# Photoroom/datago

Hardware: AMD Instinct MI355X
Metric: Mpixel/s device-resident JPEG decode+bucket-resize at 1/2/4/8 MI355X (higher is better)
Workload: dtype u8

## Files before the change

datago_amd/csrc/dg_entropy.h:

```cpp
#pragma once
#include "dg_pixel.h"
#include "dg_plane.h"
#include "dg_types.h"

namespace dg {

DG_HD int32_t huff_extend(int32_t v, int32_t s) { return v < (1 << (s - 1)) ? v - (1 << s) + 1 : v; }

DG_HD uint32_t bswap32(uint32_t x) {
  return (x >> 24) | ((x >> 8) & 0xFF00u) | ((x << 8) & 0xFF0000u) | (x << 24);
}

DG_HD uint32_t ds_word_index(uint32_t w, uint32_t lsw) {
  const uint32_t s = w >> lsw, j = w & ((1u << lsw) - 1u);
  return ((((s >> 6) << lsw) + j) << 6) + (s & 63u);
}
DG_HD uint64_t ds_words_alloc(uint32_t nsub, uint32_t lsw) {
  const uint32_t margin = ((1024u >> 5) >> lsw) + 2u;
  return ((uint64_t)((nsub + margin + 63u) / 64u) << lsw) * 64;
}

constexpr uint32_t kBwBuf = 6;

struct BitWin {
// ... 98 lines not shown
      eob = 1;
      break;
    }
    const uint32_t nadv = adv + (size == 0u ? 16u : run + 1u);
    if (nadv > 64u) break;
    adv = nadv;
    o += len + size;
    if (adv == 64u) break;
  }
  return o | (adv << 4) | (eob << 11);
}

DG_HD uint32_t multi_next_z(uint32_t m, uint32_t z) {
  const uint32_t c = m & 15u, adv = (m >> 4) & 127u, eob = (m >> 11) & 1u;
  const bool ok = c != 0u && z != 0u && (eob ? z + adv < 64u : z + adv <= 64u);
  return ok ? (eob ? 64u : z + adv) : 0xFFFFFFFFu;
}

struct RangeAcc {
  uint32_t out;
  uint32_t m, n;
  int32_t dc[3];
};

struct WriteCtx {
  int16_t *blk;
  uint32_t sw = 0;
  DG_GLOBAL int16_t *coef;
  uint32_t seg, nin;
  int32_t pred[3];
  uint32_t blocks_per_seg, total_blocks;
  int32_t cur;
  uint32_t zs;
#if defined(DG_DEVICE)
  DG_GLOBAL uint8_t *cnt = nullptr;
  int16_t *wave_blk;
  uint32_t stride;
  uint32_t *tab;
  const ImageDesc *im;
  const int32_t *qt;
  const uint8_t *n2z;
  BatchFlags *flags;
  uint32_t img;
#endif
};

DG_HD int32_t wc_index(const WriteCtx &w, uint32_t in_seg) {
  if (w.blocks_per_seg && in_seg >= w.blocks_per_seg) return -1;
  uint64_t g = (uint64_t)(w.blocks_per_seg ? w.seg : 0) * w.blocks_per_seg + in_seg;
  return g < w.total_blocks ? (int32_t)g : -1;
}

DG_HD void wc_begin(WriteCtx &w, int32_t idx, uint32_t zs) {
  w.cur = idx;
  w.zs = zs;
#if defined(DG_DEVICE)
  u32x4 *p = (u32x4 *)w.blk;
  const u32x4 zero = {0u, 0u, 0u, 0u};
#pragma unroll
  for (int i = 0; i < 8; i++) p[i] = zero;
#else
  for (int i = 0; i < 64; i++) w.blk[i] = 0;
#endif
}

DG_HD void wc_flush(WriteCtx &w, uint32_t ze) {
  if (w.cur < 0) return;
  DG_GLOBAL int16_t *dst = w.coef + (size_t)w.cur * 64;
  if (w.zs == 0 && ze == 64) {
#if defined(DG_DEVICE)
    const u32x4 *s4 = (const u32x4 *)w.blk;
    DG_GLOBAL u32x4 *d4 = (DG_GLOBAL u32x4 *)dst;
#pragma unroll
    for (int i = 0; i < 8; i++) d4[i] = s4[i ^ (w.sw >> 3)];
#else
    for (int i = 0; i < 64; i++) dst[i] = w.blk[i ^ w.sw];
#endif
  } else {
    for (uint32_t i = w.zs; i < ze; i++) dst[i] = w.blk[i ^ w.sw];
  }
#if defined(DG_DEVICE)
  if (w.cnt) w.cnt[w.cur] = 0xFFu;
#endif
  w.cur = -1;
}

#if defined(DG_DEVICE)
__device__ __forceinline__ void wc_list_late(WriteCtx &w, int32_t idx) {
  if (!w.im || idx < 0) return;
  const uint32_t e = atomicAdd(&w.flags->idct_late, 1u);
  if (e < w.flags->idct_cap) {
    uint32_t *l = (uint32_t *)(uintptr_t)w.flags->idct_list;
    l[2 * e] = w.img;
    l[2 * e + 1] = (uint32_t)idx;
  }
}

__device__ __forceinline__ void wc_coop_flush(WriteCtx &w, bool pending) {
  const uint64_t pm = __ballot(pending);
  if (!pm) return;
  const uint64_t am = __ballot(1);
  if (pending) {
    const uint32_t rank = __builtin_amdgcn_mbcnt_hi((uint32_t)(pm >> 32), __builtin_amdgcn_mbcnt_lo((uint32_t)pm, 0u));
    w.tab[rank] = __lane_id();
    w.tab[64 + rank] = (uint32_t)w.cur;
  }
  __builtin_amdgcn_wave_barrier();
  const uint32_t wr = __builtin_amdgcn_mbcnt_hi((uint32_t)(am >> 32), __builtin_amdgcn_mbcnt_lo((uint32_t)am, 0u));
  const uint32_t na = (uint32_t)__popcll(am), nb = (uint32_t)__popcll(pm), nc = 8u * nb;
  const u32x4 zero = {0u, 0u, 0u, 0u};
  if (w.im && na >= 8) {
    const ImageDesc &im = *w.im;
    const bool zune = im.sem != 0;
    const uint32_t groups = na >> 3, g = wr >> 3, part = wr & 7u;
    for (uint32_t k0 = 0; k0 < nb; k0 += groups) {
      const uint32_t k = k0 + g;
      const bool act = g < groups && k < nb;
      const int32_t idx = act ? (int32_t)w.tab[64 + k] : -1;
      const uint32_t own = act ? w.tab[k] & 255u : 0u;
      int16_t *b = w.wave_blk + own * w.stride;
      const uint32_t osw = w.stride == 64u ? ((own >> 1) & 7u) << 3 : 0u;
      const bool live = act && idx >= 0;
      uint32_t c = 0, by = 0, bx = 0;
      if (live) block_pos(im, (uint32_t)idx, c, by, bx);
      int32_t ws[8];
      if (live) {
        int32_t v[8];
#pragma unroll
        for (int r = 0; r < 8; r++) v[r] = (int32_t)b[w.n2z[r * 8 + part] ^ osw] * w.qt[c * 64 + r * 8 + part];
        idct_col(zune, v, ws);
      }
      __builtin_amdgcn_wave_barrier();
      if (live) {
#pragma unroll
        for (int r = 0; r < 8; r++) b[r * 8 + part] = (int16_t)ws[r];
      }
      __builtin_amdgcn_wave_barrier();
      if (act) {
        u32x4 *row4 = (u32x4 *)b + part;
        if (live) {
          const u32x4 rv = *row4;
          int16_t h[8];
          __builtin_memcpy(h, &rv, 16);
          int32_t row[8];
          uint32_t px[8];
#pragma unroll
          for (int i = 0; i < 8; i++) row[i] = h[i];
          idct_row(zune, row, px);
          store_plane_row8(im, c, by * 8 + part, bx, px);
        }
        *row4 = zero;
      }
      __builtin_amdgcn_wave_barrier();
    }
    return;
  }
  for (uint32_t c = wr; c < nc; c += na) {
    const uint32_t k = c >> 3, part = c & 7u;
    const int32_t idx = (int32_t)w.tab[64 + k];
    const uint32_t own = w.tab[k] & 255u;
    u32x4 *src = (u32x4 *)(w.wave_blk + own * w.stride) + (w.stride == 64u ? part ^ ((own >> 1) & 7u) : part);
    const u32x4 v = *src;
    const bool nz = (v.x | v.y | v.z | v.w) != 0u;
    if (idx >= 0 && (nz || !w.cnt)) *(DG_GLOBAL u32x4 *)(w.coef + (size_t)idx * 64 + part * 8) = v;
    if (w.cnt && nz) atomicOr(&w.tab[k], 256u << part);
    *src = zero;
    if (part == 0) wc_list_late(w, idx);
  }
  __builtin_amdgcn_wave_barrier();
  if (w.cnt && wr < nb) {
    const int32_t idx = (int32_t)w.tab[64 + wr];
    if (idx >= 0) w.cnt[idx] = (uint8_t)(w.tab[wr] >> 8);
  }
  __builtin_amdgcn_wave_barrier();
}

__device__ __forceinline__ void wc_flush_zero(WriteCtx &w, uint32_t ze) {
  wc_flush(w, ze);
  u32x4 *p = (u32x4 *)w.blk;
  const u32x4 zero = {0u, 0u, 0u, 0u};
#pragma unroll
  for (int i = 0; i < 8; i++) p[i] = zero;
}
#endif

template <bool COOP>
DG_HD void wc_end_block(WriteCtx &w, bool &pending) {
// ... 282 lines not shown
    const int32_t v = huff_value(bits, len, size);
    uint32_t zm = 0xFFFFFFFFu, mc = 0;
    if (!WRITE) {
      const uint32_t m = (mi != 3u && !isdc) ? (uint32_t)mt[(mi << kMultiBits) | (bits >> (32u - kMultiBits))] : 0u;
      mc = m & 15u;
      zm = pos + mc <= ev ? multi_next_z(m, z) : 0xFFFFFFFFu;
    }
    const bool take_m = zm != 0xFFFFFFFFu;
    pos += take_m ? mc : len + size;
    const int32_t vdc = isdc ? v : 0;
    acc.n += isdc ? 1u : 0u;
    add3(acc.dc, comp, vdc);
    if (stage) {
      if (isdc) {
        stg->started++;
        if (v) stage_push(*stg, stage_coef(0, stg->started, v));
      } else if (size && z + run < 64) {
        stage_push(*stg, stage_coef(z + run, stg->started, v));
      }
    }
    if (WRITE) {
      add3(w->pred, comp, vdc);
      if (isdc) {
        if (COOP) {
          w->cur = wc_index(*w, w->nin);
          w->zs = 0;
        } else {
          wc_begin(*w, wc_index(*w, w->nin), 0);
        }
        w->nin++;
      }
      const uint32_t zz = z + run;
      if (isdc || (size && zz < 64u)) w->blk[zz ^ w->sw] = (int16_t)(isdc ? sel3(w->pred, comp) : v);
    }
    uint32_t zn = take_m ? zm : huff_next_z(z, sym);
    if (pair && !stage && (WRITE || !take_m)) {
      uint32_t used = len + size;
      bool open = isdc || !(size == 0u && run != 15u);
#pragma unroll
      for (uint32_t x = 0; x < 3u; x++) {
        if (x >= pair) break;
        const uint32_t bx = used < 32u ? bits << used : 0u;
        const uint32_t ex = huff_decode(*tac, bx);
        const uint32_t lx = ex >> 8, sx = ex & 0xFFu, zx = sx & 15u;
        const bool tk = open && zn < 64u && pos < ev && used + lx + zx <= 32u;
        if (tk) {
          if (WRITE) {
            const uint32_t zz2 = zn + (sx >> 4);
            if (zx && zz2 < 64u) w->blk[zz2 ^ w->sw] = (int16_t)huff_value(bx, lx, zx);
          }
          pos += lx + zx;
          used += lx + zx;
          zn = huff_next_z(zn, sx);
        }
        open = tk && !(zx == 0u && (sx >> 4) != 15u);
      }
    }
    bw_shift(b, pos);
    const bool bend = zn >= 64u;
    if (WRITE && bend) wc_end_block<COOP>(*w, pending);
    z = bend ? 0u : zn;
    r = bend ? (r + 1u == bpm ? 0u : r + 1u) : r;
    comp = (cbits >> (2u * r)) & 3u;
    block_tables(tdc, tac);
  }
  if (WRITE && z > 0) wc_partial<COOP>(*w, z);
  if (stage) stage_finish(*stg);
  if (!merged) {
    uint32_t rel = pos - a1;
    acc.out = pack_state(rel > 255 ? 255 : rel, r, z);
  }
  for (uint32_t j = 0; j < k; j++) {
    DG_GLOBAL Ckpt &c = ck[j];
    if (acc.m > c.m) {
      c.m = acc.m - c.m;
      c.n = acc.n;
      c.dc[0] = acc.dc[0];
      c.dc[1] = acc.dc[1];
      c.dc[2] = acc.dc[2];
    } else {
      c.m = 0;
      c.n = acc.n - c.n;
// ... 242 lines not shown
```

datago_amd/csrc/dg_types.h:

```cpp
#pragma once
#include <stdint.h>

#if defined(__HIP__)
#define DG_HD __host__ __device__ __forceinline__
#define DG_DEVICE 1
#define DG_GLOBAL __attribute__((address_space(1)))
typedef unsigned int u32x4 __attribute__((ext_vector_type(4)));
typedef unsigned int u32x2 __attribute__((ext_vector_type(2)));
#else
#define DG_HD static inline
#define DG_GLOBAL
#endif

namespace dg {

template <class T>
DG_HD DG_GLOBAL T *gp(uint64_t a) {
  return (DG_GLOBAL T *)(uintptr_t)a;
}

DG_HD int32_t sel3(const int32_t v[3], uint32_t c) { return c == 0 ? v[0] : (c == 1 ? v[1] : v[2]); }
DG_HD void add3(int32_t v[3], uint32_t c, int32_t d) {
  v[0] += c == 0 ? d : 0;
  v[1] += c == 1 ? d : 0;
// ... 10 lines not shown
constexpr int kSubBits = 16 - kLutBits;
constexpr int kMaxSubTables = 8;
struct HuffTable {
  uint16_t lut[1 << kLutBits];
  uint16_t sub[kMaxSubTables][1 << kSubBits];
  uint32_t lim[17];
  int32_t valoff[17];
  uint8_t vals[256];
};

struct QuantTable {
  uint16_t q[64];
};

DG_HD uint32_t pack_state(uint32_t rel, uint32_t r, uint32_t z) {
  return 0x80000000u | (rel << 16) | (r << 8) | z;
}
DG_HD uint32_t st_rel(uint32_t s) { return (s >> 16) & 0xFFu; }
DG_HD uint32_t st_r(uint32_t s) { return (s >> 8) & 0xFFu; }
DG_HD uint32_t st_z(uint32_t s) { return s & 0xFFu; }

struct SubState {
  uint32_t in;
  uint32_t out;
  uint32_t m;
  uint32_t n;
  int32_t dc[3];
  uint32_t seg;
  uint32_t nin;
  int32_t dcin[3];
  uint32_t nstart;
  uint32_t nent;
};

enum Colorspace : uint32_t { CS_YCC = 0, CS_RGB = 1, CS_GRAY = 2 };

struct ResizePass {
  uint64_t src, dst;
  uint64_t coef;
  uint64_t bounds;
  double in0, in1;
  uint32_t in_size, out_size;
  uint32_t ksize;
  int32_t precision;
  uint32_t src_stride, dst_stride;
  uint32_t width, rows;
  uint32_t out0;
  uint32_t bands;
  uint32_t row0;
  uint32_t C;
  uint32_t kind;
  uint32_t mode;
};
constexpr uint32_t kHFused = 1, kHDirect = 2;
constexpr uint32_t kHVFused = 4;
constexpr uint32_t kHDecode = 8, kHDecWide = 16;
constexpr uint32_t kDecCols = 128;
constexpr uint32_t kDecSeg0 = 320, kDecSeg1 = 640;
constexpr uint32_t kDecStripsDefault = 8;
constexpr uint32_t kHVSegPx = 320;
constexpr uint32_t kHVTapsMax = 24;
constexpr uint32_t kHVRows = 64;
constexpr uint32_t kHBandRows = 8;
constexpr uint32_t kHBandCols = 128;
constexpr uint32_t kIdctItemStride = 4;

// ... 109 lines not shown
  uint64_t scan;
  uint32_t scan_len;
  uint32_t nsub;
  uint32_t sub_base;
  uint32_t sub_bits;
  uint32_t ckpt_base;
  uint64_t ds;
  uint64_t mk;
  uint64_t chunk;
  uint32_t nchunk;
  uint32_t ds_state0;
  uint32_t ds_bits;
  uint32_t nmk;
  uint32_t slotmap;
  uint32_t mk_cap;
  uint32_t lead_bits;
  uint32_t ds_lsw;
  uint32_t ckpt;
  uint32_t idct_fused;
  uint32_t stage_cap;
  uint32_t restart;
  uint32_t blocks_per_seg;
  uint32_t total_blocks;
  uint32_t bpm;
  uint32_t comp_bits;
  uint8_t blk_comp[12];
  uint16_t hslot[kMaxSlots];
  uint8_t ncomp, colorspace, dec_c, nslots;
  uint16_t qpool[3];
  uint16_t sem;
  uint64_t coef;
  uint64_t stage;
  uint64_t ccnt;
  uint32_t width, height;
  uint32_t mcux, mcuy;
  uint32_t hmax, vmax;
  uint32_t ch[3], cv[3];
  uint32_t cfirst[3];
  uint32_t cbw[3], cbh[3];
  uint32_t cdsw[3], cdsh[3];
  uint64_t plane[3];
  uint64_t pix;
  uint32_t pix_stride;
  int32_t status;
  ResizePass pass[kStages];
  uint64_t out;
  uint32_t out_w, out_h, out_c, out_stride;
  uint64_t final_src;
  uint32_t final_src_stride, copy_needed;
  uint32_t final_src_c;
  uint32_t color_fused;
  uint32_t fmt;
  uint32_t prog;
  uint32_t crec;
  uint32_t copy_mode;
  PngDesc png;
  AlphaOp aop[kAlphaPoints];
  EncDesc enc;
};

struct ProgScan {
  uint64_t data;
  uint32_t len;
  uint32_t image;
  uint32_t ns;
  uint32_t comp[4];
// ... 42 lines not shown
```

datago_amd/csrc/host/pipeline.cpp:

```cpp
#include "pipeline.h"

#include <string.h>

#include <algorithm>
#include <time.h>
#include <atomic>
#include <chrono>
#include <cmath>
#include <thread>

#include "../dg_entropy.h"
#include "../dg_pixel.h"
#include "../kernels.h"

namespace dg {

thread_local std::string g_last_error;
void set_error(const std::string &s) { g_last_error = s; }

#define HIPCHK(x)                                                                          \
  do {                                                                                     \
    hipError_t e_ = (x);                                                                   \
    if (e_ != hipSuccess) {                                                                \
      set_error(std::string("HIP error: ") + hipGetErrorString(e_) + " at " #x);          \
// ... 492 lines not shown
    return DG_OK;
  }
  if (k == "prog_pipe") {
    prog_pipe_ = v != 0;
    return DG_OK;
  }
  if (k == "prog_serial") {
    prog_serial_ = v != 0;
    return DG_OK;
  }
  if (k == "entropy_once") {
    entropy_once_ = v != 0;
    return DG_OK;
  }
  if (k == "entropy_lpt") {
    entropy_lpt_ = v != 0;
    return DG_OK;
  }
  if (k == "hb_bands") {
    if (v < 1 || v > 64) return opt_error(k, v, "valid unless v < 1 || v > 64");
    hb_bands_ = (uint32_t)v;
    return DG_OK;
  }
  if (k == "idct_fused") {
    idct_fused_ = v != 0;
    return DG_OK;
  }
  if (k == "idct_thread") {
    idct_thread_ = v != 0;
    return DG_OK;
  }
  if (k == "sparse_coef") {
    sparse_coef_ = v != 0;
    return DG_OK;
  }
  if (k == "h_prefetch") {
    h_prefetch_ = v != 0;
    return DG_OK;
  }
  if (k == "h_planar") {
    h_planar_ = v != 0;
    return DG_OK;
  }
  if (k == "destuff_one") {
    destuff_one_ = v != 0;
    return DG_OK;
  }
  if (k == "chroma_rec") {
    chroma_rec_ = v != 0;
    return DG_OK;
  }
  if (k == "reset_host_us") {
    for (double &x : host_us_) x = 0;
    for (double &x : host_cpu_us_) x = 0;
    return DG_OK;
  }
  if (k == "hv_fused") {
    hv_fused_ = v != 0;
    return DG_OK;
  }
  if (k == "copy_threads") {
    if (v < 1 || v > 64) return opt_error(k, v, "valid unless v < 1 || v > 64");
    copy_threads_ = (int)v;
    return DG_OK;
  }
  if (k == "ckpt") {
// ... 870 lines not shown
  ccache_maybe_reset(sl);
  struct CacheRoll {
    Context *c;
    size_t n0, off0;
    bool armed = true;
    ~CacheRoll() {
      if (armed) c->ccache_rollback(n0, off0);
    }
  } croll{this, ccache_.size(), ccache_off_};
  uint32_t sub_bits = sub_bits_;
  bool small = false;
  if (!sub_bits) {
    uint64_t coded = 0;
    for (int i = 0; i < n; i++)
      if (!b.plans[i].status && b.plans[i].fmt == kFmtJpeg && !b.plans[i].hdr.progressive)
        coded += b.plans[i].hdr.scan_end - b.plans[i].hdr.scan_off;
    small = coded < small_coded_;
    sub_bits = coded >= (64ull << 20) ? sub_auto_ : small ? sub_small_ : 2048u;
  }
  last_sub_bits_ = sub_bits;
  Layout L;
  Layout CO;
  Layout IN;
  Layout LT, CH;
  const bool alias = png_alias_;
  std::vector<size_t> in_off(n, 0);
  size_t out_total = 0;
  uint64_t ckpt_total = 0;
  b.out_dev_off.assign(n, 0);
  b.out_direct.assign(n, 0);
  uint32_t sub_base = 0;
  b.descs.reserve(n);
  struct Offs {
    size_t coef, ccnt, plane[3], pix, pass_dst[kStages], pass_coef[kStages], pass_bounds[kStages], pass_srcoff[kStages];
    int pass_cache[kStages];
    bool pass_hit[kStages];
    size_t final_off, tmp, out, ds, mk, chunk, stage;
    size_t zs, raw, unf, pal;
    size_t tout, ecoef, ebits, ewords, hdr, eaux;
    int aop_stage[kAlphaPoints];
    size_t aop_off[kAlphaPoints];
    uint32_t late = 0;
    int img = -1;
  };
  std::vector<Offs> offs;
  for (int i = 0; i < n; i++) {
    ImagePlan &p = b.plans[i];
    if (p.status) continue;
    ImageDesc d;
    memset(&d, 0, sizeof(d));
    Offs o;
    memset(&o, 0, sizeof(o));
    o.late = 0;
    o.img = i;
    for (int s_ = 0; s_ < kStages; s_++) o.pass_cache[s_] = -1;
    uint32_t W, H, C;
    size_t cur_stride;
    bool colour = false;
    if (p.fmt == kFmtPng) {
      const PngHeader &g = p.png;
      W = g.width;
      H = g.height;
      C = (uint32_t)g.out_c;
      d.fmt = kFmtPng;
      d.width = W;
      d.height = H;
      d.dec_c = (uint8_t)C;
// ... 126 lines not shown
        d.sub_bits = sub_bits / 4;
      else if (bpb < sub_density_ && sub_bits >= 1024)
        d.sub_bits = sub_bits / 2;
    }
    d.idct_fused = (idct_fused_ && !entropy_once_) ? 1u : 0u;
    if (write_split_ && d.ckpt && !d.idct_fused && !entropy_once_ && h.restart == 0 && d.sub_bits >= 1024 &&
        d.sub_bits / 2 / kCkptBits - 1 < num_ckpt(d.sub_bits))
      d.ckpt |= 2u;
    if (d.idct_fused) b.any_fused = true;
    d.lead_bits = lead_bits_ >= 0 ? (uint32_t)lead_bits_ : small ? lead_small_ : (bpm >= 4 ? lead_big_ : 2048u);
    if (lead_density_ && lead_bits_ < 0 && d.sub_bits < sub_bits)
      d.lead_bits = std::max<uint32_t>(1024u, d.lead_bits / (sub_bits / d.sub_bits));
    d.nsub = std::max<uint32_t>(1, (uint32_t)(((uint64_t)d.scan_len * 8 + d.sub_bits - 1) / d.sub_bits));
    d.sub_base = sub_base;
    sub_base += d.nsub;
    d.ckpt_base = (uint32_t)ckpt_total;
    ckpt_total += (uint64_t)d.nsub * num_ckpt(d.sub_bits);
    d.nchunk = std::max<uint32_t>(1, (d.scan_len + kDestuffChunk - 1) / kDestuffChunk);
    uint32_t mcus = h.ncomp == 1 ? d.total_blocks : d.mcux * d.mcuy;
    d.mk_cap = (d.restart ? mcus / d.restart + 2 : 0) + 64;
    d.ds_lsw = 0;
    while ((32u << d.ds_lsw) < d.sub_bits) d.ds_lsw++;
    o.ds = L.take((size_t)ds_words_alloc(d.nsub, d.ds_lsw) * 4, 256);
    if (entropy_once_ && d.sub_bits <= 8192) {
      d.stage_cap = (d.sub_bits / 2 + d.sub_bits / 8 + 64 + 3) / 4;
      o.stage = L.take((size_t)((d.nsub + 63) / 64) * d.stage_cap * 64 * 16, 256);
      b.stage_on = true;
    }
    o.mk = L.take((size_t)d.mk_cap * 4, 16);
    o.chunk = L.take((size_t)d.nchunk * 16, 16);
    if (host_io) in_off[i] = IN.take(lens[i] + 16, 16);
    }
    o.coef = CO.take((size_t)d.total_blocks * 128);
    o.ccnt = (sparse_coef_ && idct_thread_ && !d.prog && !d.idct_fused && !entropy_once_)
                 ? CO.take((size_t)d.total_blocks, 64) + 1
                 : 0;
    for (int c = 0; c < 3; c++) o.plane[c] = (size_t)-1;
    C = d.dec_c;
    colour = h.ncomp == 3;
    if (h.ncomp == 3) {
      d.pix_stride = (uint32_t)align_up((size_t)W * 3, 16);
      cur_stride = d.pix_stride;
    } else {
      cur_stride = (size_t)d.cbw[0] * 8;
    }
    }
    d.out_w = p.out_w;
    d.out_h = p.out_h;
    d.out_c = p.out_c;
    d.out_stride = p.out_w * p.out_c;
    uint32_t cw = W, chh = H;
    uint32_t xoff = 0, yoff = 0;
    int last_stage = -1;
    auto add_pass = [&](int stage, uint32_t kind, double in0, double in1, uint32_t in_size, uint32_t out_size,
                        uint32_t out0, uint32_t width, uint32_t rows, uint32_t row0) -> ResizePass & {
      ResizePass &ps = d.pass[stage];
      ps.kind = kind;
      ps.in0 = in0;
      ps.in1 = in1;
      ps.in_size = in_size;
      ps.out_size = out_size;
      ps.out0 = out0;
      ps.ksize = fir_ksize(in0, in1, out_size);
      ps.src_stride = (uint32_t)cur_stride;
      ps.width = width;
      ps.rows = rows;
      ps.row0 = row0;
      ps.bands = hb_bands_;
      ps.C = C;
// ... 278 lines not shown
    d.out = out;
    if (d.enc.active) {
      EncDesc &e = d.enc;
      e.src = out;
      e.out = user_out;
      e.coef = (uint64_t)(uintptr_t)(S + o.ecoef);
      e.bits = (uint64_t)(uintptr_t)(S + o.ebits);
      e.words = (uint64_t)(uintptr_t)(S + o.ewords);
      e.aux = o.eaux ? (uint64_t)(uintptr_t)(S + o.eaux) : 0;
      e.hdr = o.hdr + 1;
    }
    if (d.fmt == kFmtPng) {
      const PngHeader &g = b.plans[i].png;
      PngDesc &pd = d.png;
      pd.zs = (uint64_t)(uintptr_t)(S + o.zs);
      pd.raw = (uint64_t)(uintptr_t)(S + o.raw);
      pd.unf = (uint64_t)(uintptr_t)(S + o.unf);
      d.pix = pd.expand ? (uint64_t)(uintptr_t)(S + o.pix) : pd.unf;
      pd.pal = g.ctype == 3 ? o.pal + 1 : 0;
      uint64_t zo = 0;
      for (size_t c = 0; c < g.idat_off.size(); c++) {
        GatherJob j;
        j.src = (uint64_t)(uintptr_t)(src + g.idat_off[c]);
        j.dst = pd.zs + zo;
        j.len = g.idat_len[c];
        j.pad = 0;
        zo += g.idat_len[c];
        b.gjobs.push_back(j);
      }
    } else {
    d.scan = (uint64_t)(uintptr_t)(src + h.scan_off);
    d.coef = (uint64_t)(uintptr_t)((char *)sl.coef.p + o.coef);
    d.ccnt = (o.ccnt && !(d.pass[0].mode & kHDecode)) ? (uint64_t)(uintptr_t)((char *)sl.coef.p + o.ccnt - 1) : 0;
    if (d.prog) {
      const size_t first = b.pscans.size();
      for (size_t j = 0; j < h.scans.size(); j++) {
        const JpegScan &sc = h.scans[j];
        ProgScan r;
        memset(&r, 0, sizeof(r));
        r.data = (uint64_t)(uintptr_t)(src + sc.off);
        r.len = (uint32_t)(sc.end - sc.off);
        r.image = (uint32_t)b.desc_of[i];
        r.ns = (uint32_t)sc.ns;
        for (int q = 0; q < sc.ns; q++) {
          r.comp[q] = (uint32_t)sc.comp[q];
          r.dc[q] = sc.dc_tab[q] >= 0 ? (uint16_t)pool_huff(h.tables[sc.dc_tab[q]]) : 0;
        }
        r.ac = sc.ac_tab >= 0 ? (uint16_t)pool_huff(h.tables[sc.ac_tab]) : 0;
        r.ss = (uint32_t)sc.ss;
        r.se = (uint32_t)sc.se;
        r.ah = (uint32_t)sc.ah;
        r.al = (uint32_t)sc.al;
        r.restart = (uint32_t)sc.restart;
        r.first = (uint32_t)first;
        r.next = kProgNoScan;
        r.pflags = 0;
        uint32_t lvl = 0;
        for (size_t e = 0; e < j; e++) {
          const JpegScan &pr = h.scans[e];
          if (pr.se < sc.ss || sc.se < pr.ss) continue;
          bool share = false;
          for (int x = 0; x < pr.ns; x++)
            for (int y = 0; y < sc.ns; y++) share |= pr.comp[x] == sc.comp[y];
          if (share) {
            lvl = std::max(lvl, b.pscans[first + e].level + 1);
            if (h.scans.size() <= kProgMaxDepScans) r.deps |= 1ull << e;
// ... 1244 lines not shown
```

datago_amd/csrc/host/pipeline.h:

```cpp
#pragma once
#include <hip/hip_runtime.h>

#include <chrono>
#include <memory>
#include <condition_variable>
#include <mutex>
#include <string>
#include <unordered_map>
#include <vector>

#include "../../../include/datago_hip.h"
#include "../dg_types.h"
#include "buckets.h"
#include "jpeg_header.h"
#include "png_header.h"
#include "jpeg_enc.h"
#include "host_pool.h"

namespace dg {

struct DevBuf {
  void *p = nullptr;
  size_t cap = 0;
};
// ... 352 lines not shown
  uint32_t sub_auto_ = 8192;
  int64_t lead_bits_ = -1;
  uint32_t last_sub_bits_ = kDefaultSubBits;
  bool timing_ = false;
  bool side_stream_ = true;
  int debug_flags_ = 0;
  bool wg_timing_ = false;
  bool chunked_off_ = false;
  uint32_t inf_chunk_ = kInfChunk;
  uint32_t inf_cap_ = 30;
  bool png_alias_ = true;
  uint32_t inf_pad_ = 65536;
  uint32_t inf_stage3_ = 32;
  int plan_threads_ = 4;
  int meta_pull_ = 1;
  size_t list_hint_[L_COUNT] = {};
  bool write_split_ = true;
  uint32_t lead_big_ = 4096;
  uint64_t small_coded_ = 0;
  uint32_t sub_small_ = 512, lead_small_ = 1024;
  uint32_t v_tile_ = 4;
  uint32_t v_units_ = 2;
  static constexpr int kPlanGrain = 32;
  std::unique_ptr<HostPool> plan_pool_;
  uint32_t hb_bands_ = kHBandsDefault;
  int decode_sem_ = 0;
  bool ckpt_ = true;
  double host_us_[8] = {0, 0, 0, 0, 0, 0, 0, 0};
  double host_cpu_us_[7] = {0, 0, 0, 0, 0, 0, 0};
  size_t last_meta_bytes_ = 0;
  int copy_threads_ = 8;
  bool hv_fused_ = false;
  bool idct_thread_ = true;
  bool sparse_coef_ = true;
  bool h_prefetch_ = true;
  bool h_planar_ = true;
  bool destuff_one_ = false;
  bool chroma_rec_ = true;
  bool band_dec_ = false;
  uint32_t uf_units_ = 1;
  uint32_t inf_decode_ = 25;
  bool h_mfma_ = false;
  double sub_density_ = 0;
  bool lead_density_ = false;
  uint32_t dec_dbg_ = 0;
  uint32_t dec_strips_ = kDecStripsDefault;
  bool idct_fused_ = false;
  bool progressive_ = true;
  bool prog_serial_ = false;
  bool prog_pipe_ = true;
  int prog_chain_ = 100;
  bool entropy_lpt_ = true;
  bool entropy_once_ = false;
  int64_t stat_png_serial_ = 0, stat_png_chunks_ = 0, stat_png_small_ = 0;
  int64_t stat_band_dec_ = 0;
  double wgstat_[2][4] = {{0}};
  int64_t stat_batches_ = 0, stat_resync_ = 0, stat_fix_ = 0, stat_mismatch_ = 0, stat_iters_ = 0;
  int64_t stat_unsettled_ = 0, stat_pool_flush_ = 0;
  int64_t stat_prog_items_ = 0, stat_prog_chains_ = 0;
  std::vector<float> last_ms_;
  std::mutex reg_mu_;
  std::vector<std::pair<uintptr_t, size_t>> registered_;
  int64_t stat_direct_d2h_ = 0;
};

}
// ... 1 lines not shown
```

datago_amd/csrc/kernels.hip:

```cpp
#include <hip/hip_runtime.h>

#include "dg_entropy.h"
#include "dg_pixel.h"
#include "dg_plane.h"
#include "kernels.h"

#pragma clang fp contract(off)

namespace dg {


__device__ __forceinline__ void load_tables(HuffTable *tabs, const HuffTable *pool, const ImageDesc &im) {
  const int words = (int)(sizeof(HuffTable) / 4);
  const int ns = im.nslots;
  for (int i = threadIdx.x; i < ns * words; i += blockDim.x) {
    int s = i / words, w = i - s * words;
    ((uint32_t *)&tabs[s])[w] = ((const uint32_t *)&pool[im.hslot[s]])[w];
  }
}


struct Destuff16 {
  uint32_t kept, mks;
  uint32_t km, mm;
// ... 691 lines not shown
      const uint32_t S = im.sub_bits, mid = s * S + S / 2, kmid = S / 2 / kCkptBits - 1;
      const Ckpt c = ckpt[im.ckpt_base + (size_t)s * num_ckpt(S) + kmid];
      const bool ok = mid < im.ds_bits && im.nmk == 0 && ss.m == 0 && c.m == 0 && st_rel(c.st) < 255u;
      if (!ok) {
        run = half == 0;
      } else if (half == 0) {
        a1o = mid;
        want = c.st;
      } else {
        a0o = mid;
        in = c.st;
        ss.nin += ss.n - c.n;
        ss.dcin[0] += ss.dc[0] - c.dc[0];
        ss.dcin[1] += ss.dc[1] - c.dc[1];
        ss.dcin[2] += ss.dc[2] - c.dc[2];
      }
    }
  }
  if (run) {
    WriteCtx w;
    w.blk = blk[t];
    w.sw = (((uint32_t)t >> 1) & 7u) << 3;
    w.coef = gp<int16_t>(im.coef);
    w.seg = ss.seg;
    w.nin = ss.nin;
    w.pred[0] = ss.dcin[0];
    w.pred[1] = ss.dcin[1];
    w.pred[2] = ss.dcin[2];
    w.blocks_per_seg = im.blocks_per_seg;
    w.total_blocks = im.total_blocks;
    w.cur = -1;
    w.zs = 0;
    w.cnt = (im.ccnt && !fused) ? gp<uint8_t>(im.ccnt) : nullptr;
    w.wave_blk = blk[t & ~63];
    w.stride = kBlkStride;
    w.tab = wtab[t >> 6];
    w.im = fused ? &im : nullptr;
    w.qt = qt;
    w.n2z = n2z;
    w.flags = flags;
    w.img = it.image;
    {
      u32x4 *p = (u32x4 *)w.blk;
      const u32x4 zero = {0u, 0u, 0u, 0u};
#pragma unroll
      for (int i = 0; i < 8; i++) p[i] = zero;
    }
    RangeAcc acc;
    decode_range<true, HuffTable, true>(im, tabs, gp<const uint8_t>(im.ds), gp<const uint32_t>(im.mk), s, in,
                                        acc, &w, nullptr, false, 0, nullptr, nullptr, 0xFFu, pair, a0o, a1o);
    if (acc.out != want || (s == 0 && (flags->debug & kDbgForceWriteMismatch))) {
      atomicAdd(&flags->write_mismatch, 1u);
      if (imgs[it.image].status == 0) imgs[it.image].status = 1;
    }
  }
  if (flags->wgtime) {
    __syncthreads();
    wg_time_store(flags, flags->wgtime_write + blockIdx.x, t_start);
  }
}

__global__ __launch_bounds__(256) void k_huff_scatter(const ImageDesc *__restrict__ imgs,
                                                      const WgItem *__restrict__ list,
                                                      const SubState *__restrict__ subs) {
  __shared__ __attribute__((aligned(16))) int16_t blk[kSubPerWg][kBlkStride];
  const WgItem it = list[blockIdx.x];
// ... 195 lines not shown
    if (item < n) break;
    item -= n;
  }
  if (c >= im.ncomp) return false;
  const uint32_t ck = (im.cbw[c] + kIdctBlocks - 1) / kIdctBlocks;
  const uint32_t by = item / ck, chunk = item - by * ck;
  const uint32_t cbw = im.cbw[c];
  const uint32_t bx = chunk * kIdctBlocks + threadIdx.x;
  const uint32_t chc = im.ch[c];
  uint32_t bidx;
  if (im.ncomp == 1) {
    bidx = by * cbw + bx;
  } else {
    const uint32_t my = by / im.cv[c], vy = by - my * im.cv[c];
    const uint32_t mx = chc == 1 ? bx : chc == 2 ? bx >> 1 : bx / chc, hx = bx - mx * chc;
    bidx = (my * im.mcux + mx) * im.bpm + im.cfirst[c] + vy * chc + hx;
  }
  L.c = c;
  L.by = by;
  L.bx = bx;
  L.v = bx < cbw;
  L.bidx = L.v ? bidx : 0u;
  return true;
}

__device__ __forceinline__ uint32_t idct_t_parts(const ImageDesc &im, const IdctLoc &L) {
  if (!L.v) return 0u;
  if (!im.ccnt) return 0xFFu;
  return gp<const uint8_t>(im.ccnt)[L.bidx];
}

__device__ __forceinline__ void idct_t_item(const ImageDesc &im, const IdctLoc &L, const u32x4 w[8],
                                            const QuantTable *__restrict__ qpool);

__global__ __launch_bounds__(64) void k_idct_t(const ImageDesc *__restrict__ imgs, const WgItem *__restrict__ list,
                                              const QuantTable *__restrict__ qpool) {
  const WgItem it = list[blockIdx.x];
  const ImageDesc &im = imgs[it.image];
  IdctLoc L;
  bool ok = idct_t_locate(im, it.item0, L);
  uint32_t np = ok ? idct_t_parts(im, L) : 0u;
#pragma nounroll
  for (uint32_t k = 0; k < kIdctItemStride && ok; k++) {
    u32x4 w[8];
    const DG_GLOBAL u32x4 *src = (const DG_GLOBAL u32x4 *)(gp<const int16_t>(im.coef) + (size_t)L.bidx * 64);
#pragma unroll
    for (uint32_t i = 0; i < 8; i++) w[i] = (np >> i) & 1u ? src[i] : u32x4{0, 0, 0, 0};
    IdctLoc N;
    const bool nok = k + 1 < kIdctItemStride && idct_t_locate(im, it.item0 + k + 1, N);
    const uint32_t nnp = nok ? idct_t_parts(im, N) : 0u;
    idct_t_item(im, L, w, qpool);
    L = N;
    ok = nok;
    np = nnp;
  }
}

__device__ __forceinline__ void idct_t_item(const ImageDesc &im, const IdctLoc &L, const u32x4 w[8],
                                            const QuantTable *__restrict__ qpool) {
  const uint32_t c = L.c, by = L.by, bx = L.bx;
  const bool v = L.v;
  const uint32_t lane = threadIdx.x, cbw = im.cbw[c];
  const bool zune = im.sem != 0;
  const DG_GLOBAL uint16_t *q = gp<const uint16_t>((uint64_t)(uintptr_t)qpool[im.qpool[c]].q);
  int32_t x[64];
  {
#pragma unroll
    for (int k = 0; k < 64; k++) {
      const uint32_t word = w[k >> 3][(k >> 1) & 3];
      const int32_t z = (int32_t)(int16_t)(k & 1 ? word >> 16 : word & 0xFFFFu);
      const int nat = kZigzagToNatural[k];
      x[nat] = __mul24(z, (int32_t)q[nat]);
    }
  }
#pragma unroll
  for (int col = 0; col < 8; col++) {
    int32_t in[8], o[8];
#pragma unroll
    for (int r = 0; r < 8; r++) in[r] = x[r * 8 + col];
    idct_col(zune, in, o);
#pragma unroll
    for (int r = 0; r < 8; r++) x[r * 8 + col] = o[r];
  }
  const bool rec = plane_is_rec(im, c);
  const int32_t e = rec ? (int32_t)crec_lim(im, c) - 1 - (int32_t)(bx * 8) : 7;
  DG_GLOBAL uint8_t *plane = gp<uint8_t>(im.plane[c]);
#pragma unroll
  for (int r = 0; r < 8; r++) {
    uint32_t px[8];
    idct_row(zune, x + r * 8, px);
    const uint32_t y = by * 8 + (uint32_t)r;
    if (!rec) {
      if (v)
        *(DG_GLOBAL u32x2 *)(plane + (size_t)y * (cbw * 8) + bx * 8) =
            u32x2{pack4(px[0], px[1], px[2], px[3]), pack4(px[4], px[5], px[6], px[7])};
      continue;
    }
    uint32_t vv[8];
    crec_clamp(e, px, vv);
    const uint32_t l = (uint32_t)__shfl_up((int)vv[7], 1), rr = (uint32_t)__shfl_down((int)vv[0], 1);
    if (v) {
      const bool have_l = lane > 0 || bx == 0, have_r = (lane + 1 < 64u && bx + 1 < cbw) || bx + 1 == cbw;
      store_crec_pair(crec_row(im, c, y), bx, cbw, vv, lane > 0 ? l : vv[0], bx + 1 < cbw ? rr : vv[7], have_l,
                      have_r);
    }
  }
}
// ... 1899 lines not shown
```

Measured before the change: 128,100.

## Store JPEG coefficients as packed int8 blocks with wide fallback

```diff
diff --git a/datago_amd/csrc/dg_entropy.h b/datago_amd/csrc/dg_entropy.h
--- a/datago_amd/csrc/dg_entropy.h
+++ b/datago_amd/csrc/dg_entropy.h
@@ -154,6 +154,8 @@
   uint32_t blocks_per_seg, total_blocks;
   int32_t cur;
   uint32_t zs;
+  DG_GLOBAL uint8_t *coef8 = nullptr;
+  uint32_t ncat = 0;
 #if defined(DG_DEVICE)
   DG_GLOBAL uint8_t *cnt = nullptr;
   int16_t *wave_blk;
@@ -189,6 +191,17 @@
 DG_HD void wc_flush(WriteCtx &w, uint32_t ze) {
   if (w.cur < 0) return;
   DG_GLOBAL int16_t *dst = w.coef + (size_t)w.cur * 64;
+  if (w.coef8) {
+    DG_GLOBAL uint8_t *d8 = w.coef8 + (size_t)w.cur * 64;
+#if !defined(DG_DEVICE)
+    if (w.zs == 0 && ze == 64 && w.ncat <= kNarrowMaxCat && narrow_dc_ok(w.blk[w.sw])) {
+      narrow_pack(w.blk, w.sw, d8);
+      w.cur = -1;
+      return;
+    }
+#endif
+    d8[63] = (uint8_t)kNarrowWide;
+  }
   if (w.zs == 0 && ze == 64) {
 #if defined(DG_DEVICE)
     const u32x4 *s4 = (const u32x4 *)w.blk;
@@ -222,9 +235,16 @@
   const uint64_t pm = __ballot(pending);
   if (!pm) return;
   const uint64_t am = __ballot(1);
+  bool wide = false;
   if (pending) {
     const uint32_t rank = __builtin_amdgcn_mbcnt_hi((uint32_t)(pm >> 32), __builtin_amdgcn_mbcnt_lo((uint32_t)pm, 0u));
-    w.tab[rank] = __lane_id();
+    uint32_t e = __lane_id();
+    if (w.coef8) {
+      const int32_t dc = w.blk[w.sw];
+      wide = w.ncat > kNarrowMaxCat || !narrow_dc_ok(dc);
+      e |= (wide ? 256u : 0u) | ((((uint32_t)dc >> 8) & 15u) << 12);
+    }
+    w.tab[rank] = e;
     w.tab[64 + rank] = (uint32_t)w.cur;
   }
   __builtin_amdgcn_wave_barrier();
@@ -275,6 +295,42 @@
       }
       __builtin_amdgcn_wave_barrier();
     }
+    return;
+  }
+  if (w.coef8) {
+    const bool anyw = __ballot(wide) != 0;
+    for (uint32_t c = wr; c < 4u * nb; c += na) {
+      const uint32_t k = c >> 2, q = c & 3u;
+      const int32_t idx = (int32_t)w.tab[64 + k];
+      const uint32_t e = w.tab[k], own = e & 255u;
+      if (e & 256u) continue;
+      u32x4 *b4 = (u32x4 *)(w.wave_blk + own * w.stride);
+      const uint32_t sx = w.stride == 64u ? (own >> 1) & 7u : 0u;
+      u32x4 *p0 = b4 + ((2u * q) ^ sx), *p1 = b4 + ((2u * q + 1u) ^ sx);
+      const u32x4 a = *p0, b = *p1;
+      constexpr uint32_t lo = 0x06040200u;
+      u32x4 o = {__builtin_amdgcn_perm(a.y, a.x, lo), __builtin_amdgcn_perm(a.w, a.z, lo),
+                 __builtin_amdgcn_perm(b.y, b.x, lo), __builtin_amdgcn_perm(b.w, b.z, lo)};
+      if (q == 3u) o.w = (o.w & 0x00FFFFFFu) | ((((b.w >> 16) & 15u) | (((e >> 12) & 15u) << 4)) << 24);
+      if (idx >= 0) *(DG_GLOBAL u32x4 *)(w.coef8 + (size_t)idx * 64 + q * 16) = o;
+      *p0 = zero;
+      *p1 = zero;
+    }
+    if (anyw) {
+      for (uint32_t c = wr; c < nc; c += na) {
+        const uint32_t k = c >> 3, part = c & 7u;
+        const int32_t idx = (int32_t)w.tab[64 + k];
+        const uint32_t e = w.tab[k], own = e & 255u;
+        if (!(e & 256u)) continue;
+        u32x4 *src = (u32x4 *)(w.wave_blk + own * w.stride) + (w.stride == 64u ? part ^ ((own >> 1) & 7u) : part);
+        if (idx >= 0) {
+          *(DG_GLOBAL u32x4 *)(w.coef + (size_t)idx * 64 + part * 8) = *src;
+          if (part == 7u) w.coef8[(size_t)idx * 64 + 63] = (uint8_t)kNarrowWide;
+        }
+        *src = zero;
+      }
+    }
+    __builtin_amdgcn_wave_barrier();
     return;
   }
   for (uint32_t c = wr; c < nc; c += na) {
@@ -623,6 +679,8 @@
       }
       const uint32_t zz = z + run;
       if (isdc || (size && zz < 64u)) w->blk[zz ^ w->sw] = (int16_t)(isdc ? sel3(w->pred, comp) : v);
+      const uint32_t nc = narrow_cat(zz, size);
+      w->ncat = isdc ? 0u : (w->ncat > nc ? w->ncat : nc);
     }
     uint32_t zn = take_m ? zm : huff_next_z(z, sym);
     if (pair && !stage && (WRITE || !take_m)) {
@@ -639,6 +697,8 @@
           if (WRITE) {
             const uint32_t zz2 = zn + (sx >> 4);
             if (zx && zz2 < 64u) w->blk[zz2 ^ w->sw] = (int16_t)huff_value(bx, lx, zx);
+            const uint32_t nc = narrow_cat(zz2, zx);
+            w->ncat = w->ncat > nc ? w->ncat : nc;
           }
           pos += lx + zx;
           used += lx + zx;
diff --git a/datago_amd/csrc/dg_types.h b/datago_amd/csrc/dg_types.h
--- a/datago_amd/csrc/dg_types.h
+++ b/datago_amd/csrc/dg_types.h
@@ -66,6 +66,31 @@
   uint32_t nstart;
   uint32_t nent;
 };
+
+constexpr uint32_t kNarrowWide = 0x8u;
+constexpr uint32_t kNarrowMaxCat = 7u;
+DG_HD uint32_t narrow_cat(uint32_t zz, uint32_t size) { return size + (zz == 63u ? 4u : 0u); }
+DG_HD bool narrow_dc_ok(int32_t dc) { return dc >= -2048 && dc <= 2047; }
+DG_HD uint32_t narrow_tail(int32_t dc, int32_t ac63) {
+  return ((uint32_t)ac63 & 15u) | ((((uint32_t)dc >> 8) & 15u) << 4);
+}
+DG_HD bool narrow_is_wide(uint32_t tail) { return (tail & 15u) == kNarrowWide; }
+DG_HD int32_t narrow_dc(uint32_t b0, uint32_t tail) {
+  return (int32_t)((tail >> 4) << 28) >> 20 | (int32_t)(b0 & 0xFFu);
+}
+DG_HD int32_t narrow_ac63(uint32_t tail) { return (int32_t)(tail << 28) >> 28; }
+DG_HD void narrow_pack(const int16_t *zz, uint32_t sw, DG_GLOBAL uint8_t *out) {
+  for (uint32_t i = 0; i < 63; i++) out[i] = (uint8_t)zz[i ^ sw];
+  out[63] = (uint8_t)narrow_tail(zz[sw], zz[63u ^ sw]);
+}
+DG_HD bool narrow_unpack(const DG_GLOBAL uint8_t *in, int16_t *zz) {
+  const uint32_t tail = in[63];
+  if (narrow_is_wide(tail)) return false;
+  zz[0] = (int16_t)narrow_dc(in[0], tail);
+  for (uint32_t i = 1; i < 63; i++) zz[i] = (int16_t)(int8_t)in[i];
+  zz[63] = (int16_t)narrow_ac63(tail);
+  return true;
+}
 
 enum Colorspace : uint32_t { CS_YCC = 0, CS_RGB = 1, CS_GRAY = 2 };
 
@@ -241,6 +266,7 @@
   uint64_t coef;
   uint64_t stage;
   uint64_t ccnt;
+  uint64_t coef8;
   uint32_t width, height;
   uint32_t mcux, mcuy;
   uint32_t hmax, vmax;
diff --git a/datago_amd/csrc/host/pipeline.cpp b/datago_amd/csrc/host/pipeline.cpp
--- a/datago_amd/csrc/host/pipeline.cpp
+++ b/datago_amd/csrc/host/pipeline.cpp
@@ -548,6 +548,10 @@
   }
   if (k == "sparse_coef") {
     sparse_coef_ = v != 0;
+    return DG_OK;
+  }
+  if (k == "narrow_coef") {
+    narrow_coef_ = v != 0;
     return DG_OK;
   }
   if (k == "h_prefetch") {
@@ -1484,7 +1488,7 @@
   uint32_t sub_base = 0;
   b.descs.reserve(n);
   struct Offs {
-    size_t coef, ccnt, plane[3], pix, pass_dst[kStages], pass_coef[kStages], pass_bounds[kStages], pass_srcoff[kStages];
+    size_t coef, ccnt, coef8, plane[3], pix, pass_dst[kStages], pass_coef[kStages], pass_bounds[kStages], pass_srcoff[kStages];
     int pass_cache[kStages];
     bool pass_hit[kStages];
     size_t final_off, tmp, out, ds, mk, chunk, stage;
@@ -1677,9 +1681,9 @@
     if (host_io) in_off[i] = IN.take(lens[i] + 16, 16);
     }
     o.coef = CO.take((size_t)d.total_blocks * 128);
-    o.ccnt = (sparse_coef_ && idct_thread_ && !d.prog && !d.idct_fused && !entropy_once_)
-                 ? CO.take((size_t)d.total_blocks, 64) + 1
-                 : 0;
+    const bool thread_path = idct_thread_ && !d.prog && !d.idct_fused && !entropy_once_;
+    o.coef8 = (narrow_coef_ && thread_path) ? CO.take((size_t)d.total_blocks * 64, 128) + 1 : 0;
+    o.ccnt = (sparse_coef_ && thread_path && !o.coef8) ? CO.take((size_t)d.total_blocks, 64) + 1 : 0;
     for (int c = 0; c < 3; c++) o.plane[c] = (size_t)-1;
     C = d.dec_c;
     colour = h.ncomp == 3;
@@ -2024,6 +2028,7 @@
     d.scan = (uint64_t)(uintptr_t)(src + h.scan_off);
     d.coef = (uint64_t)(uintptr_t)((char *)sl.coef.p + o.coef);
     d.ccnt = (o.ccnt && !(d.pass[0].mode & kHDecode)) ? (uint64_t)(uintptr_t)((char *)sl.coef.p + o.ccnt - 1) : 0;
+    d.coef8 = (o.coef8 && !(d.pass[0].mode & kHDecode)) ? (uint64_t)(uintptr_t)((char *)sl.coef.p + o.coef8 - 1) : 0;
     if (d.prog) {
       const size_t first = b.pscans.size();
       for (size_t j = 0; j < h.scans.size(); j++) {
diff --git a/datago_amd/csrc/host/pipeline.h b/datago_amd/csrc/host/pipeline.h
--- a/datago_amd/csrc/host/pipeline.h
+++ b/datago_amd/csrc/host/pipeline.h
@@ -408,6 +408,7 @@
   int copy_threads_ = 8;
   bool hv_fused_ = false;
   bool idct_thread_ = true;
+  bool narrow_coef_ = true;
   bool sparse_coef_ = true;
   bool h_prefetch_ = true;
   bool h_planar_ = true;
diff --git a/datago_amd/csrc/kernels.hip b/datago_amd/csrc/kernels.hip
--- a/datago_amd/csrc/kernels.hip
+++ b/datago_amd/csrc/kernels.hip
@@ -747,6 +747,7 @@
     w.cur = -1;
     w.zs = 0;
     w.cnt = (im.ccnt && !fused) ? gp<uint8_t>(im.ccnt) : nullptr;
+    w.coef8 = (im.coef8 && !fused) ? gp<uint8_t>(im.coef8) : nullptr;
     w.wave_blk = blk[t & ~63];
     w.stride = kBlkStride;
     w.tab = wtab[t >> 6];
@@ -1008,11 +1009,25 @@
 
 __device__ __forceinline__ void idct_t_item(const ImageDesc &im, const IdctLoc &L, const u32x4 w[8],
                                             const QuantTable *__restrict__ qpool);
+__device__ __forceinline__ void idct_t_item8(const ImageDesc &im, const IdctLoc &L, const u32x4 n[4],
+                                             const QuantTable *__restrict__ qpool);
 
 __global__ __launch_bounds__(64) void k_idct_t(const ImageDesc *__restrict__ imgs, const WgItem *__restrict__ list,
                                               const QuantTable *__restrict__ qpool) {
   const WgItem it = list[blockIdx.x];
   const ImageDesc &im = imgs[it.image];
+  if (im.coef8) {
+    IdctLoc L;
+#pragma nounroll
+    for (uint32_t k = 0; k < kIdctItemStride && idct_t_locate(im, it.item0 + k, L); k++) {
+      u32x4 n[4];
+      const DG_GLOBAL u32x4 *src = (const DG_GLOBAL u32x4 *)(gp<const uint8_t>(im.coef8) + (size_t)L.bidx * 64);
+#pragma unroll
+      for (uint32_t i = 0; i < 4; i++) n[i] = L.v ? src[i] : u32x4{0, 0, 0, 0};
+      idct_t_item8(im, L, n, qpool);
+    }
+    return;
+  }
   IdctLoc L;
   bool ok = idct_t_locate(im, it.item0, L);
   uint32_t np = ok ? idct_t_parts(im, L) : 0u;
@@ -1032,23 +1047,58 @@
   }
 }
 
+__device__ __forceinline__ void idct_t_dequant(const u32x4 w[8], const DG_GLOBAL uint16_t *q, int32_t x[64]) {
+#pragma unroll
+  for (int k = 0; k < 64; k++) {
+    const uint32_t word = w[k >> 3][(k >> 1) & 3];
+    const int32_t z = (int32_t)(int16_t)(k & 1 ? word >> 16 : word & 0xFFFFu);
+    const int nat = kZigzagToNatural[k];
+    x[nat] = __mul24(z, (int32_t)q[nat]);
+  }
+}
+
+__device__ __forceinline__ void idct_t_xform(const ImageDesc &im, const IdctLoc &L, int32_t x[64]);
+
 __device__ __forceinline__ void idct_t_item(const ImageDesc &im, const IdctLoc &L, const u32x4 w[8],
                                             const QuantTable *__restrict__ qpool) {
+  const DG_GLOBAL uint16_t *q = gp<const uint16_t>((uint64_t)(uintptr_t)qpool[im.qpool[L.c]].q);
+  int32_t x[64];
+  idct_t_dequant(w, q, x);
+  idct_t_xform(im, L, x);
+}
+
+__device__ __forceinline__ void idct_t_item8(const ImageDesc &im, const IdctLoc &L, const u32x4 n[4],
+                                             const QuantTable *__restrict__ qpool) {
+  const DG_GLOBAL uint16_t *q = gp<const uint16_t>((uint64_t)(uintptr_t)qpool[im.qpool[L.c]].q);
+  const uint32_t tail = n[3].w >> 24;
+  const bool wide = L.v && narrow_is_wide(tail);
+  int32_t x[64];
+#pragma unroll
+  for (int k = 0; k < 64; k++) {
+    const uint32_t word = n[k >> 4][(k >> 2) & 3];
+    const int32_t z = k == 0    ? narrow_dc(word, tail)
+                      : k == 63 ? narrow_ac63(tail)
+                                : (int32_t)(word << (24 - 8 * (k & 3))) >> 24;
+    const int nat = kZigzagToNatural[k];
+    x[nat] = __mul24(z, (int32_t)q[nat]);
+  }
+  if (__ballot(wide)) {
+    if (wide) {
+      u32x4 w[8];
+      const DG_GLOBAL u32x4 *src = (const DG_GLOBAL u32x4 *)(gp<const int16_t>(im.coef) + (size_t)L.bidx * 64);
+#pragma unroll
+      for (uint32_t i = 0; i < 8; i++) w[i] = src[i];
+      idct_t_dequant(w, q, x);
+    }
+  }
+  idct_t_xform(im, L, x);
+}
+
+__device__ __forceinline__ void idct_t_xform(const ImageDesc &im, const IdctLoc &L, int32_t x[64]) {
   const uint32_t c = L.c, by = L.by, bx = L.bx;
   const bool v = L.v;
   const uint32_t lane = threadIdx.x, cbw = im.cbw[c];
   const bool zune = im.sem != 0;
-  const DG_GLOBAL uint16_t *q = gp<const uint16_t>((uint64_t)(uintptr_t)qpool[im.qpool[c]].q);
-  int32_t x[64];
-  {
-#pragma unroll
-    for (int k = 0; k < 64; k++) {
-      const uint32_t word = w[k >> 3][(k >> 1) & 3];
-      const int32_t z = (int32_t)(int16_t)(k & 1 ? word >> 16 : word & 0xFFFFu);
-      const int nat = kZigzagToNatural[k];
-      x[nat] = __mul24(z, (int32_t)q[nat]);
-    }
-  }
 #pragma unroll
   for (int col = 0; col < 8; col++) {
     int32_t in[8], o[8];
```

Result: no change. 127,900 (-0.1%).
